# openai/whisper

Hardware: AMD Instinct MI355X
Metric: audio-seconds transcribed per wall-second (large-v3 greedy) (higher is better)
Workload: dtype f16

## Files before the change

### whisper_amd/csrc/api.cpp

```cpp
#include "../../include/whisper_hip.h"
#include "kernels.h"
#include "flac_core.h"

#include <hip/hip_runtime.h>
#include <math.h>
#include <cmath>
#include <stdlib.h>
#include <string.h>
#include <atomic>
#include <mutex>
#include <new>
#include <vector>

using namespace whk;

static thread_local hipError_t g_last_hip = hipSuccess;

#define HIPCHK(expr)                                   \
  do {                                                 \
    hipError_t _e = (expr);                            \
    if (_e != hipSuccess) { g_last_hip = _e; return WH_ERR_HIP; } \
  } while (0)

extern "C" int wh_abi_version(void) { return WH_ABI_VERSION; }
extern "C" const char* wh_status_string(int s) {
  switch (s) {
    case WH_OK: return "ok";
    case WH_ERR_ARG: return "invalid argument";
    case WH_ERR_WORKSPACE: return "workspace too small";
    case WH_ERR_HIP: return "HIP runtime error";
    case WH_ERR_STATE: return "invalid call sequence";
    case WH_ERR_LIMIT: return "compiled-in limit exceeded";
    case WH_ERR_HANDOFF: return "in-kernel hand-off timed out (results invalid)";
    case WH_RUNNING: return "loop still running (call wh_task_poll again)";
    case WH_ERR_STREAM: return "the FLAC stream fails its checks";
    default: return "unknown status";
  }
}
extern "C" int wh_last_hip_error(void) { return (int)g_last_hip; }
extern "C" const char* wh_last_hip_error_string(void) { return hipGetErrorString(g_last_hip); }

static inline size_t align_up(size_t x, size_t a) { return (x + a - 1) / a * a; }

struct Carver {
  char* base; size_t off;
  explicit Carver(void* b) : base((char*)b), off(0) {}
  void* take(size_t bytes) {
    off = align_up(off, 256);
    void* p = base ? base + off : nullptr;
    off += bytes;
    return p;
  }
};

struct wh_model {
  wh_dims d;
  int dtype;
  int esize;
  int kc1;
  wh_model_weights w;
  std::vector<wh_layer_weights> enc, dec;
};

static std::mutex g_tab_mutex;
static float* g_mel_tables[64] = {nullptr};

static int mel_tables(float** out) {
  int dev = 0;
  HIPCHK(hipGetDevice(&dev));
  if (dev < 0 || dev >= 64) return WH_ERR_ARG;
  std::lock_guard<std::mutex> lock(g_tab_mutex);
  if (!g_mel_tables[dev]) {
    std::vector<float> h(1200);
    const double PI = 3.14159265358979323846;
    for (int i = 0; i < 400; ++i) {
      h[i] = (float)cos(2.0 * PI * i / 400.0);
      h[400 + i] = (float)sin(2.0 * PI * i / 400.0);
      h[800 + i] = (float)(0.5 - 0.5 * cos(2.0 * PI * i / 400.0));
    }
    float* d = nullptr;
    HIPCHK(hipMalloc((void**)&d, 1200 * sizeof(float)));
    HIPCHK(hipMemcpy(d, h.data(), 1200 * sizeof(float), hipMemcpyHostToDevice));
    g_mel_tables[dev] = d;
  }
  *out = g_mel_tables[dev];
  return WH_OK;
}

extern "C" int wh_log_mel(const float* audio, int64_t n_samples, int batch, int n_mels,
                          const float* filters, float* out, void* scratch, void* stream) {
  if (!audio || !filters || !out || !scratch) return WH_ERR_ARG;
  if (n_samples <= 200 || batch <= 0 || n_mels <= 0 || n_mels > 128) return WH_ERR_ARG;
  if (n_samples / 160 <= 0) return WH_ERR_ARG;
  float* tables = nullptr;
  int rc = mel_tables(&tables);
  if (rc != WH_OK) return rc;
  HIPCHK(launch_log_mel(audio, n_samples, batch, n_mels, filters, tables, out, scratch, (hipStream_t)stream));
  return WH_OK;
}

extern "C" int wh_model_create(const wh_dims* dims, int dtype, const wh_model_weights* weights, wh_model** out) {
  if (!dims || !weights || !out) return WH_ERR_ARG;
  if (dtype != WH_F32 && dtype != WH_F16) return WH_ERR_ARG;
  const wh_dims& d = *dims;
  if (d.n_audio_state != d.n_text_state) return WH_ERR_ARG;
  if (d.n_audio_state % 64 != 0 || d.n_audio_state / 64 != d.n_audio_head || d.n_text_state / 64 != d.n_text_head)
    return WH_ERR_ARG;
  if (d.n_audio_state > 2048 || d.n_mels > 128 || d.n_audio_ctx > 1536 || d.n_text_ctx > 1536) return WH_ERR_LIMIT;
  if (weights->flags & ~(WH_WEIGHTS_DEC_LN_FOLDED | WH_WEIGHTS_ENC_QK_SCALED)) return WH_ERR_ARG;
  if (dtype == WH_F32 && weights->flags != 0) return WH_ERR_ARG;
  wh_model* m = new (std::nothrow) wh_model();
  if (!m) return WH_ERR_ARG;
  m->d = d;
  m->dtype = dtype;
  m->esize = dtype == WH_F16 ? 2 : 4;
  m->kc1 = (int)align_up((size_t)3 * d.n_mels, 64);
  m->w = *weights;
  m->enc.assign(weights->enc_layers, weights->enc_layers + d.n_audio_layer);
  m->dec.assign(weights->dec_layers, weights->dec_layers + d.n_text_layer);
  m->w.enc_layers = m->enc.data();
  m->w.dec_layers = m->dec.data();
  *out = m;
  return WH_OK;
}
extern "C" void wh_model_destroy(wh_model* m) { delete m; }

static hipError_t gemm(const wh_model* m, const void* A, int64_t lda, const void* W, int K, void* C, int64_t ldc,
                       int M, int N, const float* bias, int act, const float* res, int64_t ldr, bool out_f32,
                       hipStream_t s) {
  GemmArgs g;
  memset(&g, 0, sizeof(g));
  g.A = A; g.lda = lda; g.W = W; g.ldw = K; g.C = C; g.ldc = ldc;
  g.bias = bias; g.act = act; g.res = res; g.ldr = ldr;
  g.M = M; g.N = N; g.K = K;
  return launch_gemm(g, m->dtype, out_f32 || m->dtype == WH_F32, 1, s);
}

struct EncWs {
  void *melT, *c1, *xn, *qkv, *vt, *att, *h;
  float* x;
  size_t total;
};
static const int VT_LD = 1536;

static EncWs enc_carve(const wh_model* m, int B, void* base) {
  const wh_dims& d = m->d;
  const size_t es = m->esize, T = d.n_audio_ctx, F = 2 * T, D = d.n_audio_state;
  Carver c(base);
  EncWs w;
  w.melT = c.take(((size_t)B * (F + 2) * d.n_mels + 256) * es);
  w.c1 = c.take(((size_t)B * (F + 2) * D + 256) * es);
  w.x = (float*)c.take((size_t)B * T * D * 4);
  w.xn = c.take((size_t)B * T * D * es);
  w.qkv = c.take((size_t)B * T * 3 * D * es);
  w.vt = m->dtype == WH_F16 ? c.take((size_t)B * D * VT_LD * es) : nullptr;
  w.att = c.take((size_t)B * T * D * es);
  w.h = c.take((size_t)B * T * 4 * D * es);
  w.total = align_up(c.off, 256);
  return w;
}

extern "C" size_t wh_encoder_workspace_bytes(const wh_model* m, int batch) {
  if (!m || batch <= 0) return 0;
  return enc_carve(m, batch, nullptr).total;
}

extern "C" int wh_encode(const wh_model* m, const void* mel, int mel_is_f16, int B, void* out, void* workspace,
                         size_t workspace_bytes, void* stream_) {
  if (!m || !mel || !out || !workspace || B <= 0) return WH_ERR_ARG;
  hipStream_t s = (hipStream_t)stream_;
  const wh_dims& d = m->d;
  const int T = d.n_audio_ctx, F = 2 * T, D = d.n_audio_state, H = d.n_audio_head, NM = d.n_mels;
  const size_t es = m->esize;
  EncWs w = enc_carve(m, B, workspace);
// ... 365 lines not shown
  if (!p) { t->phrases_on = false; return WH_OK; }
  if (!p->child_begin || !p->child_token || !p->child_node) return WH_ERR_ARG;
  if (p->n_nodes < 2 || p->n_nodes > WH_PHRASE_MAX_NODES || p->n_edges != p->n_nodes - 1) return WH_ERR_ARG;
  if (!std::isfinite(p->boost) || p->boost == 0.f) return WH_ERR_ARG;
  if (t->needs_reset) { const int rc = task_reset_impl(t, stream); if (rc != WH_OK) return rc; }
  HIPCHK(launch_phrase_root_table(p->child_begin, p->child_token, p->child_node, p->n_edges, t->m->d.n_vocab,
                                  t->phrase_root, (hipStream_t)stream));
  t->phrases = *p;
  t->phrases_on = true;
  return WH_OK;
}

extern "C" int wh_task_set_repetition(wh_task* t, int no_repeat_ngram_size, float repetition_penalty, void* stream) {
  TASK_ENTER(t);
  if (!t) return WH_ERR_ARG;
  if (no_repeat_ngram_size < 0 || no_repeat_ngram_size > WH_REPETITION_MAX_NGRAM) return WH_ERR_ARG;
  if (!std::isfinite(repetition_penalty) || !(repetition_penalty > 0.f)) return WH_ERR_ARG;
  if (t->needs_reset) { const int rc = task_reset_impl(t, stream); if (rc != WH_OK) return rc; }
  t->rep = RepArgs{no_repeat_ngram_size, repetition_penalty};
  t->rep_on = no_repeat_ngram_size != 0 || repetition_penalty != 1.0f;
  return WH_OK;
}

static inline void* self_k_layer(const wh_task* t, int l) {
  const wh_dims& d = t->m->d;
  return (char*)t->self_k + (size_t)l * t->R * d.n_text_ctx * d.n_text_state * t->m->esize;
}
static inline void* self_v_layer(const wh_task* t, int l) {
  const wh_dims& d = t->m->d;
  return (char*)t->self_v + (size_t)l * t->R * d.n_text_ctx * d.n_text_state * t->m->esize;
}
static inline int64_t cross_ld(const wh_task* t) { return 2 * (int64_t)t->m->d.n_text_state; }
static inline int64_t cross_bs(const wh_task* t) { return (int64_t)t->m->d.n_audio_ctx * cross_ld(t); }
static inline void* cross_layer(const wh_task* t, int l) {
  return (char*)t->cross_kv + (size_t)l * t->B * cross_bs(t) * t->m->esize;
}
static inline void* cross_v_layer(const wh_task* t, int l) {
  return (char*)cross_layer(t, l) + (size_t)t->m->d.n_text_state * t->m->esize;
}
static inline int64_t cross_vt_bs(const wh_task* t) { return (int64_t)t->m->d.n_text_state * t->vt_ld; }
static inline void* cross_vt_layer(const wh_task* t, int l) {
  return (char*)t->cross_vt + (size_t)l * t->B * cross_vt_bs(t) * t->m->esize;
}

extern "C" int wh_task_set_audio(wh_task* t, const void* features, void* stream_) {
  TASK_ENTER(t);
  if (!t || !features) return WH_ERR_ARG;
  if (t->needs_reset) { const int rc = task_reset_impl(t, stream_); if (rc != WH_OK) return rc; }
  hipStream_t s = (hipStream_t)stream_;
  const wh_model* m = t->m;
  const wh_dims& d = m->d;
  const int D = d.n_text_state, Ta = d.n_audio_ctx, M = t->B * Ta;
  const size_t es = m->esize;
  for (int l = 0; l < d.n_text_layer; ++l) {
    const wh_layer_weights& L = m->dec[l];
    HIPCHK(gemm(m, features, D, L.ckv_w, D, cross_layer(t, l), cross_ld(t), M, 2 * D, L.ckv_b, 0, nullptr, 0, false, s));
  }
  if (t->cross_vt) {
    for (int l = 0; l < d.n_text_layer; ++l) {
      const wh_layer_weights& L = m->dec[l];
      GemmArgs g; memset(&g, 0, sizeof(g));
      g.A = (const char*)L.ckv_w + (size_t)D * D * es; g.lda = D; g.a_bs = 0;
      g.W = features; g.ldw = D; g.w_bs = (int64_t)Ta * D;
      g.C = cross_vt_layer(t, l); g.ldc = t->vt_ld; g.c_bs = cross_vt_bs(t);
      g.bias = L.ckv_b + D; g.bias_on_m = 1;
      g.M = D; g.N = Ta; g.K = D;
      HIPCHK(launch_gemm(g, m->dtype, 0, t->B, s));
    }
  }
  t->audio_set = true;
  return WH_OK;
}


struct StepPlan { bool frag_att, frag_self, frag_mlp, tail_merge, post_cq, post_fc1; };
static StepPlan step_plan(const wh_task* t) {
  const wh_model* m = t->m;
  const int D = m->d.n_text_state, R = t->R;
  StepPlan p;
  const bool frag_on = m->dtype == WH_F16 && !WH_DEV_FLAG("WH_NO_FRAGMENT_ORDER");
  p.frag_att = frag_on && gemv8_will_run(R, D, D, PRO_PLAIN);
  p.frag_self = p.frag_att && !t->fused_sattn && !t->fused_xout && t->self_splits <= 1;
  p.frag_mlp = frag_on && (m->w.flags & WH_WEIGHTS_DEC_LN_FOLDED) && gemv8_will_run(R, 4 * D, D, PRO_LN) &&
               gemv8_will_run(R, D, 4 * D, PRO_PLAIN);
  p.tail_merge = m->dtype == WH_F16 && !t->fused_xattn && t->G == 1 && R <= 16 && t->cross_splits >= 2 &&
                 t->cross_splits <= 4 && !WH_DEV_FLAG("WH_NO_TAIL_MERGE");
  const bool post_on = m->dtype == WH_F16 && (m->w.flags & WH_WEIGHTS_DEC_LN_FOLDED) && R >= 9 && R <= 24 &&
                       !(t->flags & WH_TASK_LN_PROLOGUE) && !WH_DEV_FLAG("WH_NO_LN_POST") && !t->fused_xattn && !t->fused_sattn &&
                       !t->fused_xout;
  auto resid_gemv8 = [&](int splits) {
    return splits <= 1 ? gemv8_will_run(R, D, D, PRO_PLAIN) : splits <= 4 && gemv8_will_run(R, D, D, PRO_COMBINE);
  };
  const bool cross_merged = p.tail_merge || (R > 16 && !WH_DEV_FLAG("WH_NO_MERGE_KERNEL"));
  p.post_cq = post_on && gemv8_will_run(R, 3 * D, D, PRO_LN) && gemv8_ln_post_pays(R, D, D) && resid_gemv8(t->self_splits);
  p.post_fc1 = post_on && gemv8_will_run(R, 3 * D, D, PRO_LN) && gemv8_ln_post_pays(R, 4 * D, D) && resid_gemv8(cross_merged ? 1 : t->cross_splits);
  return p;
}

static GemvArgs ln_proj(const wh_model* m, const float* x, int rows, const float* ln_w, const float* ln_b, const void* W,
                        const float* bias, int N, int K) {
  GemvArgs g; memset(&g, 0, sizeof(g));
  g.pro = PRO_LN; g.xf = x; g.xf_ld = K; g.ln_w = ln_w; g.ln_b = ln_b; g.ln_folded = (m->w.flags & WH_WEIGHTS_DEC_LN_FOLDED) ? 1 : 0;
  g.W = W; g.bias = bias; g.N = N; g.K = K; g.R = rows;
  return g;
}
static GemvArgs ln_site(const wh_task* t, bool post, bool publish, const float* x, const float* ln_w, const float* ln_b,
                        const void* W, const float* bias, int N) {
  GemvArgs g = ln_proj(t->m, x, t->R, ln_w, ln_b, W, bias, N, t->m->d.n_text_state);
  if (post) { g.pro = PRO_LN_POST; g.xh = t->xh; }
// ... 1159 lines not shown
```

### whisper_amd/csrc/gemm.hip

```cpp
#include "common.h"
#include "kernels.h"
#include <stdlib.h>
#include <type_traits>

namespace {

template <typename OutT> struct Out4;
template <> struct Out4<float> {
  static __device__ __forceinline__ void store(float* p, float4v v) { *(float4v*)p = v; }
};
template <> struct Out4<half_t> {
  static __device__ __forceinline__ void store(half_t* p, float4v v) {
    half4v h = {(half_t)v[0], (half_t)v[1], (half_t)v[2], (half_t)v[3]};
    *(half4v*)p = h;
  }
};

__device__ __forceinline__ void order_memory_ops() { asm volatile("" ::: "memory"); }

constexpr int FM = 4, FN = 4;


constexpr int NS = 2;
template <typename T, typename OutT, int WGM, int WGN>
__global__ __launch_bounds__(WGM * WGN * 64) void gemm_nt_kernel(whk::GemmArgs p) {
  extern __shared__ __attribute__((aligned(16))) char smem[];
  typedef typename ET<T>::unit_t unit_t;
  constexpr int UNIT = ET<T>::UNIT;
  constexpr int BKE = 128 / (int)sizeof(T);
  constexpr int NW = WGM * WGN;
  constexpr int BM = WGM * FM * 16, BN = WGN * FN * 16;
  constexpr int A_BYTES = BM * 128, W_BYTES = BN * 128, STAGE_BYTES = A_BYTES + W_BYTES;
  constexpr int IA = BM / (NW * 8), IW = BN / (NW * 8);
  static_assert(IA * NW * 8 == BM && IW * NW * 8 == BN, "tile rows must split evenly over the waves");

  const int tid = threadIdx.x, lane = tid & 63;
  const int wave = __builtin_amdgcn_readfirstlane(tid >> 6);
  const int wm = wave / WGN, wn = wave % WGN;

  const int nwg = gridDim.x, orig = blockIdx.x;
  const int xcd = orig & 7, qq = nwg >> 3, rr = nwg & 7;
  const int wg = (xcd < rr ? xcd * (qq + 1) : rr * (qq + 1) + (xcd - rr) * qq) + (orig >> 3);
  const int tile_m = wg / p.tiles_n, tile_n = wg - tile_m * p.tiles_n;
  const int m0 = tile_m * BM, n0 = tile_n * BN;
  const int64_t bz = blockIdx.z;

  const T* A = (const T*)p.A + bz * p.a_bs;
  const T* W = (const T*)p.W + bz * p.w_bs;

  const T* ga[IA];
  const T* gw[IW];
#pragma unroll
  for (int i = 0; i < IA; ++i) {
    const int r = (wave * IA + i) * 8 + (lane >> 3);
    const int u = (lane & 7) ^ ((r >> 1) & 7);
    int am = m0 + r; if (am > p.M - 1) am = p.M - 1;
    ga[i] = A + (int64_t)am * p.lda + u * UNIT;
  }
// ... 101 lines not shown
    if (m >= p.M) continue;
    const int rm = (p.res_mod > 0) ? (m % p.res_mod) : m;
    const float bm = bmpre[tm];
#pragma unroll
    for (int tn = 0; tn < FN; ++tn) {
      const int n = n0 + wn * (FN * 16) + tn * 16 + (lane >> 4) * 4;
      if (n >= p.N) continue;
      float4v v = acc[tn][tm];
      v += bpre[tn];
      v[0] += bm; v[1] += bm; v[2] += bm; v[3] += bm;
      if (p.act == 1) {
#pragma unroll
        for (int e = 0; e < 4; ++e) v[e] = gelu_erf(v[e]);
      }
      if (vec_ok && n + 3 < p.N) {
        if (R) {
          const float4v r4 = *(const float4v*)(R + (int64_t)rm * p.ldr + n);
          v += r4;
        }
        Out4<OutT>::store(C + (int64_t)m * p.ldc + n, v);
      } else {
#pragma unroll
        for (int e = 0; e < 4; ++e) {
          if (n + e < p.N) {
            float x = v[e];
            if (R) x += R[(int64_t)rm * p.ldr + n + e];
            C[(int64_t)m * p.ldc + n + e] = from_f32<OutT>(x);
          }
        }
      }
    }
  }
}


constexpr int ROWS_PATCH = 2048;
constexpr int ROWS_LDS = 2 * (256 + 256) * 128 + 16 * ROWS_PATCH;
static_assert(ROWS_LDS <= 160 * 1024, "LDS ring + epilogue patches do not fit");

template <int ACT, int BIAS>
__global__ __launch_bounds__(1024) void gemm_f16_rows_kernel(whk::GemmArgs p) {
  extern __shared__ __attribute__((aligned(16))) char smem[];
  constexpr int BM = 256, BN = 256, WGN = 4;
  constexpr int A_BYTES = BM * 128, W_BYTES = BN * 128, W_BASE = 2 * A_BYTES, RING_BYTES = 2 * (A_BYTES + W_BYTES);
  constexpr int IA = 2, IW = 2, LPS = IA + IW;
  constexpr int NST = FM * 2;
  static_assert(A_BYTES + 3 * 2048 < 65536 && W_BYTES + 3 * 2048 < 65536, "ds_read offset field");

  const int tid = threadIdx.x, lane = tid & 63;
  const int wave = __builtin_amdgcn_readfirstlane(tid >> 6);
  const int wm = wave / WGN, wn = wave % WGN;

  const int nwg = gridDim.x, orig = blockIdx.x;
  int tile, tile_end, tile_step;
  {
    const int xcd = orig & 7;
    const int total = p.persistent ? p.tiles_m * p.tiles_n : nwg;
    const int qq = total >> 3, rr = total & 7;
    const int band = xcd < rr ? xcd * (qq + 1) : rr * (qq + 1) + (xcd - rr) * qq;
    tile = band + (orig >> 3);
    tile_end = p.persistent ? band + qq + (xcd < rr ? 1 : 0) : tile + 1;
    tile_step = p.persistent ? (nwg >> 3) : 1;
  }
  if (tile >= tile_end) return;
  const int64_t bz = blockIdx.z;
  const char* A = (const char*)((const half_t*)p.A + bz * p.a_bs);
  const char* W = (const char*)((const half_t*)p.W + bz * p.w_bs);
  half_t* C = (half_t*)p.C + bz * p.c_bs;
  const int nk = p.K / 64;

  auto fresh_lane = []() {
    int l;
    asm volatile("v_mbcnt_lo_u32_b32 %0, -1, 0\n\tv_mbcnt_hi_u32_b32 %0, -1, %0" : "=v"(l));
    return l;
  };
  auto opaque = [](uint32_t v) { asm volatile("" : "+v"(v)); return v; };

  int m0, n0;
  uint32_t ga[IA], gw[IW];
  auto set_tile = [&](int t) {
    const int tile_m = t / p.tiles_n, tile_n = t - tile_m * p.tiles_n;
    m0 = tile_m * BM; n0 = tile_n * BN;
    const int ln = fresh_lane();
#pragma unroll
    for (int i = 0; i < IA; ++i) {
      const int r = (wave * IA + i) * 8 + (ln >> 3);
      const int u = (ln & 7) ^ ((r >> 1) & 7);
      int am = m0 + r; if (am > p.M - 1) am = p.M - 1;
      ga[i] = (uint32_t)(((int64_t)am * p.lda + u * 8) * 2);
    }
#pragma unroll
    for (int i = 0; i < IW; ++i) {
      const int r = (wave * IW + i) * 8 + (ln >> 3);
      const int u = (ln & 7) ^ ((r >> 1) & 7);
      int wr = n0 + r; if (wr > p.N - 1) wr = p.N - 1;
      gw[i] = (uint32_t)(((int64_t)wr * p.ldw + u * 8) * 2);
    }
  };
  auto stage = [&](int buf, int kt) {
    char* sA = smem + buf * A_BYTES + (wave * IA) * 1024;
    char* sW = smem + W_BASE + buf * W_BYTES + (wave * IW) * 1024;
    const char* Ak = A + (int64_t)kt * 128;
    const char* Wk = W + (int64_t)kt * 128;
#pragma unroll
    for (int i = 0; i < IA; ++i) glds16(Ak + opaque(ga[i]), sA + i * 1024);
#pragma unroll
    for (int i = 0; i < IW; ++i) glds16(Wk + opaque(gw[i]), sW + i * 1024);
  };

  uint32_t fa[2], fw[2];
#pragma unroll
  for (int q = 0; q < 2; ++q) {
    const int su = ((4 * q + (lane >> 4)) ^ ((lane >> 1) & 7)) << 4;
    fa[q] = (wm * 64 + (lane & 15)) * 128 + su;
    fw[q] = W_BASE + (wn * 64 + (lane & 15)) * 128 + su;
  }

  WH_PROBE_AT(p, orig, 0);
  set_tile(tile);
  stage(0, 0);
  bool counted = false;
  char* patch = smem + RING_BYTES + wave * ROWS_PATCH;

  for (int visit = 0;; ++visit) {
    float bias_lane = 0.f;
    if (BIAS != 0) {
      int bi = (BIAS == 2 ? m0 + wm * 64 : n0 + wn * 64) + fresh_lane();
      const int lim = (BIAS == 2 ? p.M : p.N) - 1;
      if (bi > lim) bi = lim;
      bias_lane = p.bias[bi];
    }

    float4v acc[FN][FM];
#pragma unroll
    for (int i = 0; i < FN; ++i)
#pragma unroll
      for (int j = 0; j < FM; ++j) acc[i][j] = float4v{0.f, 0.f, 0.f, 0.f};

    if (counted) wait_vmcnt<NST>(); else wait_vmcnt<0>();
    __builtin_amdgcn_s_barrier();
    WH_PROBE_AT(p, orig, visit == 0 ? 1 : 7);
    auto mfmas = [&](auto buf_tag) {
      constexpr int BUF = decltype(buf_tag)::value;
#pragma unroll
      for (int q = 0; q < 2; ++q) {
        half8v af[FM], wf[FN];
#pragma unroll
        for (int t = 0; t < FM; ++t) af[t] = *(const half8v*)(smem + fa[q] + (BUF * A_BYTES + t * 2048));
#pragma unroll
        for (int t = 0; t < FN; ++t) wf[t] = *(const half8v*)(smem + fw[q] + (BUF * W_BYTES + t * 2048));
#pragma unroll
        for (int tn = 0; tn < FN; ++tn)
#pragma unroll
          for (int tm = 0; tm < FM; ++tm) mma16(wf[tn], af[tm], acc[tn][tm]);
      }
    };
#pragma clang loop unroll(disable)
    for (int kt = 0; kt < nk; kt += 2) {
      stage(1, kt + 1);
      mfmas(std::integral_constant<int, 0>());
      wait_vmcnt<0>();
      __builtin_amdgcn_s_barrier();
      const bool more = kt + 2 < nk;
      if (more) stage(0, kt + 2);
      mfmas(std::integral_constant<int, 1>());
      if (more) {
        wait_vmcnt<0>();
        __builtin_amdgcn_s_barrier();
      }
    }
    if (visit == 0) WH_PROBE_AT(p, orig, 2);

    const int cm0 = m0, cn0 = n0;
    const int next = tile + tile_step;
    const bool has_next = next < tile_end;
    __builtin_amdgcn_s_barrier();
    if (visit == 0) WH_PROBE_AT(p, orig, 3);
    if (has_next) {
      set_tile(next);
      stage(0, 0);
      order_memory_ops();
    }
    tile = next;

#ifdef WH_GEMM_PROBE_NOEPI
#pragma unroll
    for (int i = 0; i < FN; ++i)
#pragma unroll
      for (int j = 0; j < FM; ++j) asm volatile("" ::"v"(acc[i][j]));
    counted = false;
#else
    const int le = fresh_lane();
    const int i16 = le & 15, g4 = le >> 4;
    if (BIAS != 0) {
      *(float*)(patch + le * 4) = bias_lane;
      if (BIAS == 2) {
#pragma unroll
        for (int tm = 0; tm < FM; ++tm) {
          const float b = *(const float*)(patch + (tm * 16 + i16) * 4);
#pragma unroll
          for (int tn = 0; tn < FN; ++tn) { acc[tn][tm][0] += b; acc[tn][tm][1] += b; acc[tn][tm][2] += b; acc[tn][tm][3] += b; }
        }
      } else {
#pragma unroll
        for (int tn = 0; tn < FN; ++tn) {
          const float4v b = *(const float4v*)(patch + (tn * 16 + g4 * 4) * 4);
#pragma unroll
          for (int tm = 0; tm < FM; ++tm) acc[tn][tm] += b;
        }
      }
    }
    const bool full = cm0 + (wm + 1) * 64 <= p.M && cn0 + (wn + 1) * 64 <= p.N;
#pragma unroll
    for (int tm = 0; tm < FM; ++tm) {
#pragma unroll
      for (int tn = 0; tn < FN; ++tn) {
        float4v v = acc[tn][tm];
        if (ACT == 1) {
#pragma unroll
          for (int e = 0; e < 4; ++e) v[e] = gelu_erf_f16out(v[e]);
        }
        const half4v h = {(half_t)v[0], (half_t)v[1], (half_t)v[2], (half_t)v[3]};
        const int slot = (tn * 4 + g4) ^ ((i16 & 7) << 1);
        *(half4v*)(patch + i16 * 128 + slot * 8) = h;
      }
#pragma unroll
      for (int j = 0; j < 2; ++j) {
        const int row = j * 8 + (le >> 3), c = le & 7;
        const float4v q = *(const float4v*)(patch + row * 128 + ((c ^ (row & 7)) << 4));
        const int m = cm0 + wm * 64 + tm * 16 + row, n = cn0 + wn * 64 + c * 8;
        half_t* dst = C + (int64_t)m * p.ldc + n;
        if (m < p.M) {
          if (n + 8 <= p.N) *(float4v*)dst = q;
          else if (n + 4 <= p.N) *(float2v*)dst = float2v{q[0], q[1]};
        }
      }
    }
    counted = full;
    if (visit == 0) WH_PROBE_AT(p, orig, 5);
#endif
    if (!has_next) break;
  }
}

template <int ACT, int BIAS>
hipError_t launch_rows(const whk::GemmArgs& a, int batch, hipStream_t stream) {
  whk::g_form = WH_FORM_NAME("gemm/rows<%d,%d>", ACT, BIAS);
  whk::GemmArgs p = a;
  p.tiles_m = (p.M + 255) / 256;
  p.tiles_n = (p.N + 255) / 256;
  static whk::LdsAttr attr;
  { hipError_t e = whk::raise_dynamic_lds(attr, (const void*)gemm_f16_rows_kernel<ACT, BIAS>, ROWS_LDS); if (e != hipSuccess) return e; }
  const int dev = WH_DEV_INT("WH_GEMM_DEV");
  const int ntiles = p.tiles_m * p.tiles_n;
  p.persistent = (batch == 1 && ntiles > 256 && !(dev & 4)) ? 1 : 0;
  dim3 grid(p.persistent ? 256 : ntiles, 1, batch);
  hipLaunchKernelGGL((gemm_f16_rows_kernel<ACT, BIAS>), grid, dim3(1024), ROWS_LDS, stream, p);
  return hipGetLastError();
}

bool rows_kernel_applies(const whk::GemmArgs& a) {
  const int dev = WH_DEV_INT("WH_GEMM_DEV");
  if (dev & 1) return false;
  if (a.res || (a.ldc & 7) || (a.N & 3) || (a.c_bs & 7) || (((uintptr_t)a.C) & 15)) return false;
  if (((int64_t)a.M * a.lda + a.K) * 2 >= (1LL << 32) || ((int64_t)a.N * a.ldw + a.K) * 2 >= (1LL << 32)) return false;
  if (!(a.M >= 1024 && a.N >= 1024 && a.K % 128 == 0)) return false;
  if (a.N <= 3072 && a.K <= 3072 && (int64_t)((a.M + 255) / 256) * ((a.N + 255) / 256) < 160) return false;
  return true;
}

hipError_t launch_rows_any(const whk::GemmArgs& a, int batch, hipStream_t stream) {
  const int bias = !a.bias ? 0 : (a.bias_on_m ? 2 : 1);
  if (a.act == 1) {
    if (bias == 0) return launch_rows<1, 0>(a, batch, stream);
    return bias == 1 ? launch_rows<1, 1>(a, batch, stream) : launch_rows<1, 2>(a, batch, stream);
  }
  if (bias == 0) return launch_rows<0, 0>(a, batch, stream);
  return bias == 1 ? launch_rows<0, 1>(a, batch, stream) : launch_rows<0, 2>(a, batch, stream);
}

template <typename T, typename OutT, int WGM, int WGN>
hipError_t launch_shape(const whk::GemmArgs& a, int batch, hipStream_t stream) {
  constexpr int BM = WGM * FM * 16, BN = WGN * FN * 16;
  constexpr int LDS = NS * (BM + BN) * 128;
  static_assert(LDS <= 160 * 1024, "LDS ring does not fit");
  whk::g_form = WH_FORM_NAME("gemm/tile<%s,%s,%d,%d>", sizeof(T) == 2 ? "half" : "float", sizeof(OutT) == 2 ? "half" : "float", WGM, WGN);
  whk::GemmArgs p = a;
  p.tiles_m = (p.M + BM - 1) / BM;
  p.tiles_n = (p.N + BN - 1) / BN;
  static whk::LdsAttr attr;
  { hipError_t e = whk::raise_dynamic_lds(attr, (const void*)gemm_nt_kernel<T, OutT, WGM, WGN>, LDS); if (e != hipSuccess) return e; }
  p.serial_epilogue = WH_DEV_FLAG("WH_GEMM_SERIAL_EPILOGUE") ? 1 : 0;
  dim3 grid(p.tiles_m * p.tiles_n, 1, batch);
  hipLaunchKernelGGL((gemm_nt_kernel<T, OutT, WGM, WGN>), grid, dim3(WGM * WGN * 64), LDS, stream, p);
  return hipGetLastError();
}

template <typename T, typename OutT>
hipError_t launch_t(const whk::GemmArgs& a, int batch, hipStream_t stream) {
  const int force = WH_DEV_INT("WH_GEMM_TILE");
  auto tiles = [&](int bm, int bn) { return (int64_t)((a.M + bm - 1) / bm) * ((a.N + bn - 1) / bn) * batch; };
  const bool small_model = a.N <= 3072 && a.K <= 3072;
  const bool big = force ? force == 256 : (a.M >= 1024 && a.N >= 1024 && !(small_model && tiles(256, 256) < 160));
  if (big) return launch_shape<T, OutT, 4, 4>(a, batch, stream);
  if (force == 128 || !small_model || tiles(128, 128) >= 192 || (int64_t)a.M * a.N <= 128 * 128)
    return launch_shape<T, OutT, 2, 2>(a, batch, stream);
  if (tiles(64, 128) >= 192) return launch_shape<T, OutT, 1, 2>(a, batch, stream);
  return launch_shape<T, OutT, 1, 1>(a, batch, stream);
}

}

namespace whk {

hipError_t launch_gemm(const GemmArgs& a, int dtype, int out_f32, int batch, hipStream_t stream) {
  const int bke = dtype == 1 ? 64 : 32;
  if (a.K % bke != 0 || a.M <= 0 || a.N <= 0) return hipErrorInvalidValue;
  if (dtype == 1) {
    if (!out_f32 && rows_kernel_applies(a)) return launch_rows_any(a, batch, stream);
    return out_f32 ? launch_t<half_t, float>(a, batch, stream) : launch_t<half_t, half_t>(a, batch, stream);
  }
  return launch_t<float, float>(a, batch, stream);
}

}
```

### whisper_amd/csrc/kernels.h

```cpp
#pragma once
#include <hip/hip_runtime.h>
#include <stdint.h>

#ifdef WH_PROBE
#define WH_PROBE_FIELD long long* probe;
#define WH_PROBE_KVHS_FIELD int64_t kv_hs;
#define WH_PROBE_AT(args, wg, i) \
  do { if ((args).probe && threadIdx.x == 0) (args).probe[(size_t)(wg) * 8 + (i)] = clock64(); } while (0)
#else
#define WH_PROBE_FIELD
#define WH_PROBE_KVHS_FIELD
#define WH_PROBE_AT(args, wg, i) do {} while (0)
#endif

#ifdef WH_DEV
#include <stdlib.h>
#define WH_DEV_FLAG(name) ([] { static const bool v = [] { const char* e = getenv(name); return e && e[0] == '1'; }(); return v; }())
#define WH_DEV_INT(name) ([] { static const int v = [] { const char* e = getenv(name); return e ? atoi(e) : 0; }(); return v; }())
#else
#define WH_DEV_FLAG(name) false
#define WH_DEV_INT(name) 0
#endif

#include <atomic>
#include <stdio.h>
#include <string>
namespace whk {

extern thread_local const char* g_form;
#define WH_FORM_NAME(...) ([&] { static const std::string s_ = [&] { char b_[96]; snprintf(b_, sizeof b_, __VA_ARGS__); \
                                                                     return std::string(b_); }(); return s_.c_str(); }())

struct LdsAttr { std::atomic<int> done[64]; };
inline hipError_t raise_dynamic_lds(LdsAttr& c, const void* fn, int bytes) {
  int dev = 0;
  hipError_t e = hipGetDevice(&dev);
  if (e != hipSuccess) return e;
  if (dev < 0 || dev >= 64) return hipErrorInvalidDevice;
  if (c.done[dev].load(std::memory_order_acquire) == 1) return hipSuccess;
  e = hipFuncSetAttribute(fn, hipFuncAttributeMaxDynamicSharedMemorySize, bytes);
  if (e == hipSuccess) c.done[dev].store(1, std::memory_order_release);
  else (void)hipGetLastError();
  return e;
}


hipError_t launch_log_mel(const float* audio, int64_t n_samples, int batch, int n_mels,
                          const float* filters, const float* tables, float* out, void* scratch,
                          hipStream_t stream);

struct GemmArgs {
  const void* A; int64_t lda; int64_t a_bs;
  const void* W; int64_t ldw; int64_t w_bs;
  void* C; int64_t ldc; int64_t c_bs;
  const float* bias; int bias_on_m;
  const float* res; int64_t ldr; int64_t r_bs; int res_mod;
  int act;
  int M, N, K;
  int tiles_m, tiles_n, persistent;
  int serial_epilogue;
  WH_PROBE_FIELD
};
hipError_t launch_gemm(const GemmArgs& a, int dtype, int out_f32, int batch, hipStream_t stream);

hipError_t launch_mel_transpose(const void* mel, int mel_is_f16, int B, int n_mels, int F, void* out,
                                int dtype, hipStream_t stream);
hipError_t launch_layernorm(const float* x, int64_t ldx, const float* w, const float* b, void* out,
                            int64_t ldo, int64_t rows, int D, int dtype, hipStream_t stream);
hipError_t launch_embed(const int64_t* tokens, int64_t stride, int R, int T0, const void* tok_emb,
                        const float* pos, const int* d_offset, const int* lag, int D, int n_vocab, float* x,
                        int dtype, hipStream_t stream);
hipError_t launch_scatter_kv(const void* qkv, int R, int T0, int D, const int* d_offset, int n_ctx,
                             void* kcache, void* vcache, int dtype, hipStream_t stream);
hipError_t launch_gather_rows(const float* x, const int* sel, int n_sel, int D, float* out,
                              hipStream_t stream);
hipError_t launch_gather_cache(const void* src, void* dst, const int* src_idx, int R, int64_t row_bytes,
                               int64_t used_bytes, hipStream_t stream);
hipError_t launch_permute_groups(void* k_base, void* v_base, int n_layers, int64_t layer_bytes, int n_audio, int G,
                                 int64_t row_bytes, int64_t used_bytes, const int* src_idx, const int* copy_from,
                                 int64_t pos_bytes, hipStream_t stream);
hipError_t launch_replicate_row(void* base, int64_t layer_bytes, int n_layers, int64_t row_bytes, int src_row, int dst_row0,
                                int G, int64_t used_bytes, hipStream_t stream);
hipError_t launch_add_int(int* p, int v, hipStream_t stream);

struct AttnArgs {
  const void* q; int64_t q_ld; int64_t q_bs;
  const void* k; int64_t k_ld; int64_t k_bs;
  const void* v; int64_t v_ld; int64_t v_bs;
  void* out; int64_t o_ld; int64_t o_bs;
  int H; int Tq; int Tk;
  const int* d_len;
  int causal;
  int kv_group;
  float* qk_out;
};
hipError_t launch_attn_generic(const AttnArgs& a, int batch, int dtype, hipStream_t stream);
hipError_t launch_attn_flash_f16(const void* q, int64_t q_ld, int64_t q_bs, const void* k, int64_t k_ld,
                                 int64_t k_bs, const void* vt, int64_t vt_ld, int64_t vt_bs, void* out,
                                 int64_t o_ld, int64_t o_bs, int B, int H, int T, int prescaled, hipStream_t stream, int Tq = 0);
struct DecAttnArgs {
  const void* q; int64_t q_ld;
  const void* k; int64_t k_ld; int64_t k_bs;
  const void* v; int64_t v_ld; int64_t v_bs;
  int64_t kv_hs;
  int H; int R; int kv_group;
  int Tk; const int* d_len; int len_plus;
  const int* lag;
  int splits;
  void* out; int64_t o_ld;
  int o_frag;
  void* part_o; float* part_ml;
  int* merge_cnt;
  const void* vt; int64_t vt_ld; int64_t vt_bs;
  WH_PROBE_FIELD
};
constexpr int DEC_ATTN_MAX_SPLITS = 16;
// ... 207 lines not shown
```

### whisper_amd/csrc/ktest.cpp

```cpp
#include <string.h>

#include "kernels.h"

using namespace whk;

extern "C" {

const char* wht_last_form() { return g_form; }
void wht_clear_form() { g_form = ""; }
int wht_attn_decode_capacity(int dtype) { return attn_decode_capacity(dtype); }
int wht_gemv8_will_run(int R, int N, int K, int pro) { return gemv8_will_run(R, N, K, pro) ? 1 : 0; }
const char* wht_gemv_family(int dtype, int pro, int epi, int R, int N, int K, int64_t ld, int ln_folded, int has_bias, int splits,
                            int H, int x_frag, int y_frag) {
  static const float some_bias = 0.f;
  GemvArgs a;
  memset(&a, 0, sizeof a);
  a.pro = pro; a.epi = epi; a.R = R; a.N = N; a.K = K; a.x_ld = a.xf_ld = ld; a.ln_folded = ln_folded;
  a.bias = has_bias ? &some_bias : nullptr; a.splits = splits; a.H = H; a.x_frag = x_frag; a.y_frag = y_frag;
  return gemv_family(a, dtype);
}

int wht_gemv(int dtype, int pro, const void* x, int64_t x_ld, const float* xf, int64_t xf_ld, const float* ln_w,
             const float* ln_b, int ln_folded, const void* part_o, const float* part_ml, int splits, int H, const void* W,
             const float* bias, int N, int K, int R, int x_frag, int y_frag, int epi, void* y, int64_t y_ld, float* resid,
// ... 10 lines not shown
  return launch_gemv(a, dtype, (hipStream_t)stream);
}

int wht_gemv_ln_post(int pro, const void* x, int64_t x_ld, int x_frag, const float* xf, int64_t xf_ld, const void* part_o,
                     const float* part_ml, int splits, int H, const void* W, const float* bias, int N, int K, int R, void* xh,
                     float* xc, int y_frag, int epi, void* y, int64_t y_ld, float* resid, int64_t resid_ld, void* kcache,
                     void* vcache, int64_t cache_bs, const int* d_pos, int D, const int* lag, void* stream) {
  GemvArgs a;
  memset(&a, 0, sizeof a);
  a.pro = pro; a.x = x; a.x_ld = x_ld; a.x_frag = x_frag; a.xf = xf; a.xf_ld = xf_ld; a.ln_folded = 1;
  a.part_o = part_o; a.part_ml = part_ml; a.splits = splits; a.H = H;
  a.W = W; a.bias = bias; a.N = N; a.K = K; a.R = R; a.xh = xh; a.xc = xc; a.y_frag = y_frag;
  a.epi = epi; a.y = y; a.y_ld = y_ld; a.resid = resid; a.resid_ld = resid_ld;
  a.kcache = kcache; a.vcache = vcache; a.cache_bs = cache_bs; a.d_pos = d_pos; a.D = D; a.lag = lag;
  return launch_gemv(a, 1, (hipStream_t)stream);
}
const char* wht_gemv_family_ln_post(int dtype, int pro, int epi, int R, int N, int K, int ln_folded, int has_xh, int has_xc) {
  static float some_f = 0.f;
  GemvArgs a;
  memset(&a, 0, sizeof a);
  a.pro = pro; a.epi = epi; a.R = R; a.N = N; a.K = K; a.x_ld = a.xf_ld = K; a.ln_folded = ln_folded; a.splits = 2; a.H = K / 64;
  a.xh = has_xh ? &some_f : nullptr; a.xc = has_xc ? &some_f : nullptr;
  return gemv_family(a, dtype);
}
int wht_gemv8_ln_post_pays(int R, int N, int K) { return gemv8_ln_post_pays(R, N, K) ? 1 : 0; }

int wht_merge_partials(const void* part_o, const float* part_ml, int splits, int R, int H, void* out, int64_t o_ld,
                       int dtype, int o_frag, void* stream) {
  return launch_merge_partials(part_o, part_ml, splits, R, H, out, o_ld, dtype, (hipStream_t)stream, o_frag);
}

int wht_attn_decode(int dtype, const void* q, int64_t q_ld, const void* k, int64_t k_ld, int64_t k_bs, const void* v,
                    int64_t v_ld, int64_t v_bs, int64_t kv_hs, int H, int R, int kv_group, int Tk, const int* d_len,
                    int len_plus, const int* lag, int splits, void* out, int64_t o_ld, int o_frag, void* part_o,
                    float* part_ml, int* merge_cnt, const void* vt, int64_t vt_ld, int64_t vt_bs, void* stream) {
  DecAttnArgs a;
  memset(&a, 0, sizeof a);
  a.q = q; a.q_ld = q_ld; a.k = k; a.k_ld = k_ld; a.k_bs = k_bs; a.v = v; a.v_ld = v_ld; a.v_bs = v_bs; a.kv_hs = kv_hs;
  a.H = H; a.R = R; a.kv_group = kv_group; a.Tk = Tk; a.d_len = d_len; a.len_plus = len_plus; a.lag = lag;
  a.splits = splits; a.out = out; a.o_ld = o_ld; a.o_frag = o_frag; a.part_o = part_o; a.part_ml = part_ml;
  a.merge_cnt = merge_cnt; a.vt = vt; a.vt_ld = vt_ld; a.vt_bs = vt_bs;
  return launch_attn_decode(a, dtype, (hipStream_t)stream);
}

int wht_gemm(int dtype, int out_f32, int batch, const void* A, int64_t lda, int64_t a_bs, const void* W, int64_t ldw,
             int64_t w_bs, void* C, int64_t ldc, int64_t c_bs, const float* bias, int bias_on_m, const float* res,
             int64_t ldr, int64_t r_bs, int res_mod, int act, int M, int N, int K, void* stream) {
  GemmArgs a;
  memset(&a, 0, sizeof a);
  a.A = A; a.lda = lda; a.a_bs = a_bs; a.W = W; a.ldw = ldw; a.w_bs = w_bs; a.C = C; a.ldc = ldc; a.c_bs = c_bs;
  a.bias = bias; a.bias_on_m = bias_on_m; a.res = res; a.ldr = ldr; a.r_bs = r_bs; a.res_mod = res_mod; a.act = act;
  a.M = M; a.N = N; a.K = K;
  return launch_gemm(a, dtype, out_f32, batch, (hipStream_t)stream);
}

int wht_attn_flash_f16(const void* q, int64_t q_ld, int64_t q_bs, const void* k, int64_t k_ld, int64_t k_bs,
                       const void* vt, int64_t vt_ld, int64_t vt_bs, void* out, int64_t o_ld, int64_t o_bs, int B, int H,
                       int T, int prescaled, int Tq, void* stream) {
  return launch_attn_flash_f16(q, q_ld, q_bs, k, k_ld, k_bs, vt, vt_ld, vt_bs, out, o_ld, o_bs, B, H, T, prescaled,
                               (hipStream_t)stream, Tq);
}

int wht_layernorm(const float* x, int64_t ldx, const float* w, const float* b, void* out, int64_t ldo, int64_t rows, int D,
                  int dtype, void* stream) {
  return launch_layernorm(x, ldx, w, b, out, ldo, rows, D, dtype, (hipStream_t)stream);
}

int wht_scatter_kv(const void* qkv, int R, int T0, int D, const int* d_offset, int n_ctx, void* kcache, void* vcache,
                   int dtype, void* stream) {
  return launch_scatter_kv(qkv, R, T0, D, d_offset, n_ctx, kcache, vcache, dtype, (hipStream_t)stream);
}

int wht_gather_cache(const void* src, void* dst, const int* src_idx, int R, int64_t row_bytes, int64_t used_bytes,
                     void* stream) {
  return launch_gather_cache(src, dst, src_idx, R, row_bytes, used_bytes, (hipStream_t)stream);
}

int wht_permute_groups(void* k_base, void* v_base, int n_layers, int64_t layer_bytes, int n_audio, int G, int64_t row_bytes,
                       int64_t used_bytes, const int* src_idx, const int* copy_from, int64_t pos_bytes, void* stream) {
  return launch_permute_groups(k_base, v_base, n_layers, layer_bytes, n_audio, G, row_bytes, used_bytes, src_idx, copy_from,
                               pos_bytes, (hipStream_t)stream);
}

int wht_replicate_row(void* base, int64_t layer_bytes, int n_layers, int64_t row_bytes, int src_row, int dst_row0, int G,
                      int64_t used_bytes, void* stream) {
  return launch_replicate_row(base, layer_bytes, n_layers, row_bytes, src_row, dst_row0, G, used_bytes, (hipStream_t)stream);
}

int wht_score_slice() { return SCORE_BN; }
size_t wht_score_scratch_bytes(int64_t M, int V) { return score_scratch_bytes(M, V); }
int wht_score(int dtype, const void* xn, int64_t ldx, const void* W, int64_t ldw, const int* target, int M, int K, int V,
              int v_end, float* logprob, float* top_logprob, int* top_token, void* scratch, size_t scratch_bytes,
              void* stream) {
  return launch_score(xn, ldx, W, ldw, target, M, K, V, v_end, logprob, top_logprob, top_token, scratch, scratch_bytes,
                      dtype, (hipStream_t)stream);
}

int wht_greedy_sample(const float* logits, int64_t logits_ld, int R, int V, int64_t* tokens, int64_t token_stride,
                      const int* d_ntok, const int* lag, int sample_begin, int eot, int timestamp_begin, int no_timestamps,
                      int max_initial_ts, int suppress_blank, int blank_token, const uint8_t* suppress_mask,
                      float* sum_logprobs, int64_t* step_tokens, int* d_alive_step, float* partials, size_t partials_bytes,
                      float temperature, uint64_t seed, int* row_state, int n_nodes, int n_edges, const int* child_begin,
                      const int* child_token, const int* child_node, const int* root_child, int* span, float boost,
                      void* stream) {
  if (R < 1 || V < 1 || partials_bytes < greedy_sample_scratch_bytes(R, V)) return hipErrorInvalidValue;
  SampleArgs a;
// ... 163 lines not shown
```

Baseline: 1173.

## Fuse per-layer cross-attention KV projections into one grouped persistent GEMM launch

When the decoder layers' cross-KV weights and biases sit at a uniform stride, the per-layer cross K/V projection GEMMs are issued as a single grouped launch. The persistent rows kernel walks tiles across groups and batch using a shared XCD-banded tile walk. This removes a per-layer launch and the tail underutilisation of each small GEMM, in exchange for extra per-tile pointer arithmetic. A non-uniform fallback still loops per layer, and a table-based entry point is added for tests.

```diff
diff --git a/whisper_amd/csrc/api.cpp b/whisper_amd/csrc/api.cpp
--- a/whisper_amd/csrc/api.cpp
+++ b/whisper_amd/csrc/api.cpp
@@ -60,6 +60,8 @@
   int kc1;
   wh_model_weights w;
   std::vector<wh_layer_weights> enc, dec;
+  bool ckv_uniform;
+  int64_t ckv_w_gs, ckv_b_gs;
 };
 
 static std::mutex g_tab_mutex;
@@ -120,6 +122,12 @@
   m->dec.assign(weights->dec_layers, weights->dec_layers + d.n_text_layer);
   m->w.enc_layers = m->enc.data();
   m->w.dec_layers = m->dec.data();
+  {
+    std::vector<const void*> w(d.n_text_layer), b(d.n_text_layer);
+    for (int l = 0; l < d.n_text_layer; ++l) { w[l] = m->dec[l].ckv_w; b[l] = m->dec[l].ckv_b; }
+    m->ckv_uniform = d.n_text_layer > 1 && w[0] && uniform_stride(w.data(), d.n_text_layer, m->esize, &m->ckv_w_gs) &&
+                     uniform_stride(b.data(), d.n_text_layer, 4, &m->ckv_b_gs);
+  }
   *out = m;
   return WH_OK;
 }
@@ -591,9 +599,17 @@
   const wh_dims& d = m->d;
   const int D = d.n_text_state, Ta = d.n_audio_ctx, M = t->B * Ta;
   const size_t es = m->esize;
-  for (int l = 0; l < d.n_text_layer; ++l) {
-    const wh_layer_weights& L = m->dec[l];
-    HIPCHK(gemm(m, features, D, L.ckv_w, D, cross_layer(t, l), cross_ld(t), M, 2 * D, L.ckv_b, 0, nullptr, 0, false, s));
+  if (m->ckv_uniform) {
+    GemmArgs g; memset(&g, 0, sizeof(g));
+    g.A = features; g.lda = D; g.W = m->dec[0].ckv_w; g.ldw = D; g.C = cross_layer(t, 0); g.ldc = cross_ld(t);
+    g.bias = m->dec[0].ckv_b; g.M = M; g.N = 2 * D; g.K = D;
+    g.groups = d.n_text_layer; g.w_gs = m->ckv_w_gs; g.bias_gs = m->ckv_b_gs; g.c_gs = (int64_t)t->B * cross_bs(t);
+    HIPCHK(launch_gemm(g, m->dtype, m->dtype == WH_F32, 1, s));
+  } else {
+    for (int l = 0; l < d.n_text_layer; ++l) {
+      const wh_layer_weights& L = m->dec[l];
+      HIPCHK(gemm(m, features, D, L.ckv_w, D, cross_layer(t, l), cross_ld(t), M, 2 * D, L.ckv_b, 0, nullptr, 0, false, s));
+    }
   }
   if (t->cross_vt) {
     for (int l = 0; l < d.n_text_layer; ++l) {
diff --git a/whisper_amd/csrc/gemm.hip b/whisper_amd/csrc/gemm.hip
--- a/whisper_amd/csrc/gemm.hip
+++ b/whisper_amd/csrc/gemm.hip
@@ -1,9 +1,17 @@
 #include "common.h"
 #include "kernels.h"
+#include "gemm_walk.h"
 #include <stdlib.h>
 #include <type_traits>
 
 namespace {
+
+#ifdef WH_GEMM_PROBE
+int g_gemm_dev = 0;
+#define GEMM_DEV() g_gemm_dev
+#else
+#define GEMM_DEV() WH_DEV_INT("WH_GEMM_DEV")
+#endif
 
 template <typename OutT> struct Out4;
 template <> struct Out4<float> {
@@ -211,21 +219,15 @@
   const int wm = wave / WGN, wn = wave % WGN;
 
   const int nwg = gridDim.x, orig = blockIdx.x;
-  int tile, tile_end, tile_step;
-  {
-    const int xcd = orig & 7;
-    const int total = p.persistent ? p.tiles_m * p.tiles_n : nwg;
-    const int qq = total >> 3, rr = total & 7;
-    const int band = xcd < rr ? xcd * (qq + 1) : rr * (qq + 1) + (xcd - rr) * qq;
-    tile = band + (orig >> 3);
-    tile_end = p.persistent ? band + qq + (xcd < rr ? 1 : 0) : tile + 1;
-    tile_step = p.persistent ? (nwg >> 3) : 1;
-  }
+  const whk::WalkRange walk =
+      whk::walk_range(p.persistent ? p.tiles_m * p.tiles_n * p.batch * p.groups : nwg, nwg, orig, p.persistent != 0);
+  int tile = walk.first;
+  const int tile_end = walk.end, tile_step = walk.step;
   if (tile >= tile_end) return;
-  const int64_t bz = blockIdx.z;
-  const char* A = (const char*)((const half_t*)p.A + bz * p.a_bs);
-  const char* W = (const char*)((const half_t*)p.W + bz * p.w_bs);
-  half_t* C = (half_t*)p.C + bz * p.c_bs;
+  const char* A;
+  const char* W;
+  half_t* C;
+  const float* bias;
   const int nk = p.K / 64;
 
   auto fresh_lane = []() {
@@ -238,8 +240,13 @@
   int m0, n0;
   uint32_t ga[IA], gw[IW];
   auto set_tile = [&](int t) {
-    const int tile_m = t / p.tiles_n, tile_n = t - tile_m * p.tiles_n;
-    m0 = tile_m * BM; n0 = tile_n * BN;
+    whk::WalkTile wt = whk::walk_tile(t, p.tiles_m, p.tiles_n, p.batch);
+    if (!p.persistent) wt.bz = blockIdx.z;
+    A = (const char*)((const half_t*)p.A + wt.bz * p.a_bs);
+    W = (const char*)((const half_t*)p.W + wt.bz * p.w_bs + wt.group * p.w_gs);
+    C = (half_t*)p.C + wt.bz * p.c_bs + wt.group * p.c_gs;
+    bias = p.bias + wt.group * p.bias_gs;
+    m0 = wt.tile_m * BM; n0 = wt.tile_n * BN;
     const int ln = fresh_lane();
 #pragma unroll
     for (int i = 0; i < IA; ++i) {
@@ -287,7 +294,7 @@
       int bi = (BIAS == 2 ? m0 + wm * 64 : n0 + wn * 64) + fresh_lane();
       const int lim = (BIAS == 2 ? p.M : p.N) - 1;
       if (bi > lim) bi = lim;
-      bias_lane = p.bias[bi];
+      bias_lane = bias[bi];
     }
 
     float4v acc[FN][FM];
@@ -331,6 +338,7 @@
     if (visit == 0) WH_PROBE_AT(p, orig, 2);
 
     const int cm0 = m0, cn0 = n0;
+    half_t* const cC = C;
     const int next = tile + tile_step;
     const bool has_next = next < tile_end;
     __builtin_amdgcn_s_barrier();
@@ -388,7 +396,7 @@
         const int row = j * 8 + (le >> 3), c = le & 7;
         const float4v q = *(const float4v*)(patch + row * 128 + ((c ^ (row & 7)) << 4));
         const int m = cm0 + wm * 64 + tm * 16 + row, n = cn0 + wn * 64 + c * 8;
-        half_t* dst = C + (int64_t)m * p.ldc + n;
+        half_t* dst = cC + (int64_t)m * p.ldc + n;
         if (m < p.M) {
           if (n + 8 <= p.N) *(float4v*)dst = q;
           else if (n + 4 <= p.N) *(float2v*)dst = float2v{q[0], q[1]};
@@ -408,23 +416,29 @@
   whk::GemmArgs p = a;
   p.tiles_m = (p.M + 255) / 256;
   p.tiles_n = (p.N + 255) / 256;
+  p.batch = batch;
+  p.groups = a.groups > 1 ? a.groups : 1;
+  if (p.groups == 1) p.w_gs = p.c_gs = p.bias_gs = 0;
   static whk::LdsAttr attr;
   { hipError_t e = whk::raise_dynamic_lds(attr, (const void*)gemm_f16_rows_kernel<ACT, BIAS>, ROWS_LDS); if (e != hipSuccess) return e; }
-  const int dev = WH_DEV_INT("WH_GEMM_DEV");
-  const int ntiles = p.tiles_m * p.tiles_n;
-  p.persistent = (batch == 1 && ntiles > 256 && !(dev & 4)) ? 1 : 0;
-  dim3 grid(p.persistent ? 256 : ntiles, 1, batch);
+  const int dev = GEMM_DEV();
+  const int64_t total = (int64_t)p.tiles_m * p.tiles_n * batch * p.groups;
+  if (batch < 1 || total >= (1LL << 30)) return hipErrorInvalidValue;
+  p.persistent = (p.groups > 1 || (total > 256 && !(dev & 4))) ? 1 : 0;
+  dim3 grid(p.persistent ? 256 : p.tiles_m * p.tiles_n, 1, p.persistent ? 1 : batch);
   hipLaunchKernelGGL((gemm_f16_rows_kernel<ACT, BIAS>), grid, dim3(1024), ROWS_LDS, stream, p);
   return hipGetLastError();
 }
 
-bool rows_kernel_applies(const whk::GemmArgs& a) {
-  const int dev = WH_DEV_INT("WH_GEMM_DEV");
+bool rows_kernel_applies(const whk::GemmArgs& a, int batch) {
+  const int dev = GEMM_DEV();
   if (dev & 1) return false;
   if (a.res || (a.ldc & 7) || (a.N & 3) || (a.c_bs & 7) || (((uintptr_t)a.C) & 15)) return false;
+  if (a.groups > 1 && (a.c_gs & 7)) return false;
   if (((int64_t)a.M * a.lda + a.K) * 2 >= (1LL << 32) || ((int64_t)a.N * a.ldw + a.K) * 2 >= (1LL << 32)) return false;
   if (!(a.M >= 1024 && a.N >= 1024 && a.K % 128 == 0)) return false;
-  if (a.N <= 3072 && a.K <= 3072 && (int64_t)((a.M + 255) / 256) * ((a.N + 255) / 256) < 160) return false;
+  const int64_t count = (int64_t)((a.M + 255) / 256) * ((a.N + 255) / 256) * (((dev & 2) || a.act) ? 1 : batch);
+  if (a.N <= 3072 && a.K <= 3072 && count < 160) return false;
   return true;
 }
 
@@ -472,14 +486,54 @@
 
 namespace whk {
 
+static bool grouped_in_one_launch(const GemmArgs& a, int dtype, int out_f32, int batch) {
+  return dtype == 1 && !out_f32 && rows_kernel_applies(a, batch) && !(GEMM_DEV() & 16);
+}
+
 hipError_t launch_gemm(const GemmArgs& a, int dtype, int out_f32, int batch, hipStream_t stream) {
   const int bke = dtype == 1 ? 64 : 32;
   if (a.K % bke != 0 || a.M <= 0 || a.N <= 0) return hipErrorInvalidValue;
+  const bool rows = dtype == 1 && !out_f32 && rows_kernel_applies(a, batch);
+  if (a.groups > 1 && !grouped_in_one_launch(a, dtype, out_f32, batch)) {
+    const int64_t es = dtype == 1 ? 2 : 4, cs = out_f32 ? 4 : es;
+    for (int g = 0; g < a.groups; ++g) {
+      GemmArgs one = a;
+      one.groups = 0; one.w_gs = one.c_gs = one.bias_gs = 0;
+      one.W = (const char*)a.W + g * a.w_gs * es;
+      one.C = (char*)a.C + g * a.c_gs * cs;
+      if (a.bias) one.bias = a.bias + g * a.bias_gs;
+      const hipError_t e = launch_gemm(one, dtype, out_f32, batch, stream);
+      if (e != hipSuccess) return e;
+    }
+    return hipSuccess;
+  }
   if (dtype == 1) {
-    if (!out_f32 && rows_kernel_applies(a)) return launch_rows_any(a, batch, stream);
+    if (rows) return launch_rows_any(a, batch, stream);
     return out_f32 ? launch_t<half_t, float>(a, batch, stream) : launch_t<half_t, half_t>(a, batch, stream);
   }
   return launch_t<float, float>(a, batch, stream);
 }
 
-}
+hipError_t launch_gemm_table(const GemmArgs& a, const void* const* W, const float* const* bias, void* const* C, int groups,
+                             int dtype, int out_f32, int batch, hipStream_t stream, int* launches) {
+  if (groups < 1 || !W || !C) return hipErrorInvalidValue;
+  const int64_t es = dtype == 1 ? 2 : 4, cs = out_f32 ? 4 : es;
+  GemmArgs g = a;
+  g.W = W[0]; g.C = C[0]; g.bias = bias ? bias[0] : nullptr;
+  if (groups > 1 && uniform_stride(W, groups, es, &g.w_gs) && uniform_stride((const void* const*)C, groups, cs, &g.c_gs) &&
+      (!bias || uniform_stride((const void* const*)bias, groups, 4, &g.bias_gs))) {
+    g.groups = groups;
+    if (launches) *launches = grouped_in_one_launch(g, dtype, out_f32, batch) ? 1 : groups;
+    return launch_gemm(g, dtype, out_f32, batch, stream);
+  }
+  g.groups = 0; g.w_gs = g.c_gs = g.bias_gs = 0;
+  for (int i = 0; i < groups; ++i) {
+    g.W = W[i]; g.C = C[i]; g.bias = bias ? bias[i] : nullptr;
+    const hipError_t e = launch_gemm(g, dtype, out_f32, batch, stream);
+    if (e != hipSuccess) return e;
+  }
+  if (launches) *launches = groups;
+  return hipSuccess;
+}
+
+}
diff --git a/whisper_amd/csrc/gemm_walk.h b/whisper_amd/csrc/gemm_walk.h
--- /dev/null
+++ b/whisper_amd/csrc/gemm_walk.h
@@ -0,0 +1,40 @@
+#pragma once
+
+#if defined(__HIPCC__) || defined(__CUDACC__)
+#define WH_WALK_FN __host__ __device__ __forceinline__
+#else
+#define WH_WALK_FN inline
+#endif
+
+namespace whk {
+
+constexpr int WALK_XCDS = 8;
+
+struct WalkBand { int begin, end; };
+WH_WALK_FN WalkBand walk_band(int total, int xcd) {
+  const int qq = total / WALK_XCDS, rr = total % WALK_XCDS;
+  const int begin = xcd < rr ? xcd * (qq + 1) : rr * (qq + 1) + (xcd - rr) * qq;
+  return WalkBand{begin, begin + qq + (xcd < rr ? 1 : 0)};
+}
+
+struct WalkRange { int first, end, step; };
+WH_WALK_FN WalkRange walk_range(int total, int nwg, int wg, bool persistent) {
+  const int xcd = wg % WALK_XCDS, slot = wg / WALK_XCDS;
+  const WalkBand b = walk_band(persistent ? total : nwg, xcd);
+  if (persistent) return WalkRange{b.begin + slot, b.end, nwg / WALK_XCDS};
+  return WalkRange{b.begin + slot, b.begin + slot + 1, 1};
+}
+
+struct WalkTile { int group, bz, tile_m, tile_n; };
+WH_WALK_FN WalkTile walk_tile(int t, int tiles_m, int tiles_n, int batch) {
+  const int per = tiles_m * tiles_n;
+  const int gb = t / per, r = t - gb * per;
+  WalkTile w;
+  w.group = gb / batch;
+  w.bz = gb - w.group * batch;
+  w.tile_m = r / tiles_n;
+  w.tile_n = r - w.tile_m * tiles_n;
+  return w;
+}
+
+}
diff --git a/whisper_amd/csrc/kernels.h b/whisper_amd/csrc/kernels.h
--- a/whisper_amd/csrc/kernels.h
+++ b/whisper_amd/csrc/kernels.h
@@ -57,11 +57,27 @@
   const float* res; int64_t ldr; int64_t r_bs; int res_mod;
   int act;
   int M, N, K;
-  int tiles_m, tiles_n, persistent;
+  int groups; int64_t w_gs, bias_gs, c_gs;
+  int tiles_m, tiles_n, persistent, batch;
   int serial_epilogue;
   WH_PROBE_FIELD
 };
 hipError_t launch_gemm(const GemmArgs& a, int dtype, int out_f32, int batch, hipStream_t stream);
+hipError_t launch_gemm_table(const GemmArgs& a, const void* const* W, const float* const* bias, void* const* C, int groups,
+                             int dtype, int out_f32, int batch, hipStream_t stream, int* launches);
+inline bool uniform_stride(const void* const* p, int n, int64_t elem_bytes, int64_t* stride) {
+  *stride = 0;
+  if (n < 1) return false;
+  if (!p[0]) { for (int i = 1; i < n; ++i) if (p[i]) return false; return true; }
+  if (n == 1) return true;
+  if (!p[1]) return false;
+  const int64_t d = (const char*)p[1] - (const char*)p[0];
+  if (d % elem_bytes) return false;
+  for (int i = 2; i < n; ++i)
+    if (!p[i] || (const char*)p[i] - (const char*)p[i - 1] != d) return false;
+  *stride = d / elem_bytes;
+  return true;
+}
 
 hipError_t launch_mel_transpose(const void* mel, int mel_is_f16, int B, int n_mels, int F, void* out,
                                 int dtype, hipStream_t stream);
diff --git a/whisper_amd/csrc/ktest.cpp b/whisper_amd/csrc/ktest.cpp
--- a/whisper_amd/csrc/ktest.cpp
+++ b/whisper_amd/csrc/ktest.cpp
@@ -86,6 +86,16 @@
   a.bias = bias; a.bias_on_m = bias_on_m; a.res = res; a.ldr = ldr; a.r_bs = r_bs; a.res_mod = res_mod; a.act = act;
   a.M = M; a.N = N; a.K = K;
   return launch_gemm(a, dtype, out_f32, batch, (hipStream_t)stream);
+}
+
+int wht_gemm_table(int dtype, int out_f32, int batch, const void* A, int64_t lda, int64_t a_bs, const void* const* W,
+                   int64_t ldw, int64_t w_bs, void* const* C, int64_t ldc, int64_t c_bs, const float* const* bias,
+                   int bias_on_m, int act, int M, int N, int K, int groups, int* launches, void* stream) {
+  GemmArgs a;
+  memset(&a, 0, sizeof a);
+  a.A = A; a.lda = lda; a.a_bs = a_bs; a.ldw = ldw; a.w_bs = w_bs; a.ldc = ldc; a.c_bs = c_bs;
+  a.bias_on_m = bias_on_m; a.act = act; a.M = M; a.N = N; a.K = K;
+  return launch_gemm_table(a, W, bias, C, groups, dtype, out_f32, batch, (hipStream_t)stream, launches);
 }
 
 int wht_attn_flash_f16(const void* q, int64_t q_ld, int64_t q_bs, const void* k, int64_t k_ld, int64_t k_bs,
```

After: 1174 (median of 6 runs). No clear change (+0.1%).
